# MingyuKim87/Safe_Denoiser

Hardware: AMD Instinct MI355X
Metric: images/sec (512x512, 50 steps, SD-v1.4 + repellency) (higher is better)
Workload: dtype bf16; 1 GPU; README-default end to end (safree = svf = lra = true, safree_neg_prompt_config.json:26-28): token ids -> CLIP -> SAFREE projection -> DDPM 50 steps x UNet on 3 guidance branches with per-prompt text switching + safe_denoiser.yaml repellency (kernel_fast, M=515, sigma 3.15, scale .33, margin 1.6, window 780<=t<=1000) -> VAE decode -> uint8 512x512 images; SD-v1.4 UNet / CLIP / VAE with random weigh; guidance_branches=3, text_encoder_precision=bf16x3, prompts_per_batch=64, latent_repeat=3, renoise_draws_rank0=3520, parallelism=prompt-shard x1

## Files before the change

include/sdn.h:

```cpp
#ifndef SDN_H_
#define SDN_H_

#include <stddef.h>
#include <stdint.h>

#ifdef __cplusplus
extern "C" {
#endif

#define SDN_OK            0
#define SDN_E_INVALID    -1
#define SDN_E_LAUNCH     -2
#define SDN_E_WORKSPACE  -3
#define SDN_E_ARCH       -4

int sdn_abi_version(void);
const char* sdn_device_arch_host(void);


#define SDN_REPEL_RBF     0
#define SDN_REPEL_SPARSE  1
#define SDN_QNORM_NONE    0
#define SDN_QNORM_CHANNEL 1
#define SDN_OUT_REPELLED  0
// ... 67 lines not shown
#define SDN_ACT_GEGLU_TANH 5
#define SDN_ACT_GELU      7
#define SDN_OUT_BF16      0
#define SDN_OUT_F32       1
#define SDN_OUT_F32_NCHW  2

typedef struct sdn_gemm_desc {
  int32_t M, N, K;
  int32_t a_mode;
  int32_t K1;
  int32_t Hs, Ws, Cin;
  int32_t Ho, Wo, stride;
  int32_t upsample;
  int32_t act;
  int32_t out_kind;
  int32_t rows_per_batch;
  int32_t ld_rowbias;
  int32_t ld_rowgate;
  int32_t residual_bcast;
  int32_t n_valid;
  int32_t ldc;
  int32_t asym_pad;
  int32_t split_k;
  int32_t res_pre;
  int32_t x3_out;
  int32_t f32_stream;
} sdn_gemm_desc;

int sdn_gemm_bf16(const sdn_gemm_desc* d_host, const void* a, const void* a2, const void* w,
                  const float* bias, const float* rowbias, const float* rowgate, const void* residual, void* out,
                  void* stream);
int sdn_gemm_f16(const sdn_gemm_desc* d_host, const void* a, const void* a2, const void* w,
                 const float* bias, const float* rowbias, const float* rowgate, const void* residual, void* out,
                 void* stream);

int sdn_groupnorm_bf16(const void* x, const void* x2, int32_t batch, int32_t hw, int32_t c1, int32_t c2,
                       int32_t groups, float eps, int32_t silu, const float* gamma, const float* beta,
                       void* out, float* stats_ws, void* stream);
int sdn_groupnorm_f16(const void* x, const void* x2, int32_t batch, int32_t hw, int32_t c1, int32_t c2,
                      int32_t groups, float eps, int32_t silu, const float* gamma, const float* beta,
                      void* out, float* stats_ws, void* stream);

int sdn_layernorm_bf16(const void* x, int64_t rows, int32_t c, float eps, const float* gamma,
                       const float* beta, void* out, void* stream);
int sdn_layernorm_f16(const void* x, int64_t rows, int32_t c, float eps, const float* gamma,
                      const float* beta, void* out, void* stream);

int sdn_attention_bf16(const void* q, const void* k, const void* v, void* out, int32_t batch, int32_t heads,
                       int32_t nq, int32_t nk, int32_t head_dim, int32_t ldq, int32_t ldk, int32_t ldv,
                       int32_t ldo, float scale, void* stream);
int sdn_attention_f16(const void* q, const void* k, const void* v, void* out, int32_t batch, int32_t heads,
                      int32_t nq, int32_t nk, int32_t head_dim, int32_t ldq, int32_t ldk, int32_t ldv,
                      int32_t ldo, float scale, void* stream);

typedef struct sdn_attn_segment2 {
  const void* q2; const void* k2; const void* v2; void* out2;
  int32_t n1, ldq2, ldk2, ldv2, ldo2;
} sdn_attn_segment2;
int sdn_joint_attention(int32_t dtype, const void* q, const void* k, const void* v, void* out,
                        const sdn_attn_segment2* seg2_host, int32_t batch, int32_t heads, int32_t n_total,
                        int32_t head_dim, int32_t ldq, int32_t ldk, int32_t ldv, int32_t ldo, float scale,
                        void* stream);

int sdn_layernorm_mod_bf16(const void* x, int64_t rows, int32_t c, float eps, const float* scale, const float* shift,
                           int32_t ld_mod, int32_t rows_per_batch, void* out, void* stream);
int sdn_layernorm_mod_f16(const void* x, int64_t rows, int32_t c, float eps, const float* scale, const float* shift,
                          int32_t ld_mod, int32_t rows_per_batch, void* out, void* stream);

int sdn_patchify_bf16(const float* latents, int32_t batch, int32_t c, int32_t h, int32_t w, int32_t p, void* out, void* stream);
int sdn_patchify_f16(const float* latents, int32_t batch, int32_t c, int32_t h, int32_t w, int32_t p, void* out, void* stream);
int sdn_unpatchify_f32(const float* tokens, int32_t batch, int32_t c, int32_t h, int32_t w, int32_t p, float* out, void* stream);

int sdn_conv_in_bf16(const float* latents_nchw, const void* w, const float* bias, int32_t batch, int32_t cin,
                     int32_t h, int32_t wd, int32_t cout, void* out_nhwc, void* stream);
int sdn_conv_in_f16(const float* latents_nchw, const void* w, const float* bias, int32_t batch, int32_t cin,
                    int32_t h, int32_t wd, int32_t cout, void* out_nhwc, void* stream);

int sdn_timestep_embed_bf16(float timestep, int32_t batch, int32_t dim, void* out, void* stream);
int sdn_timestep_embed_f16(float timestep, int32_t batch, int32_t dim, void* out, void* stream);

int sdn_gemm_f32(const sdn_gemm_desc* d_host, const void* a, const void* a2, const void* w,
                 const float* bias, const float* rowbias, const float* rowgate, const void* residual, void* out,
                 void* stream);
int sdn_groupnorm_f32(const void* x, const void* x2, int32_t batch, int32_t hw, int32_t c1, int32_t c2,
                      int32_t groups, float eps, int32_t silu, const float* gamma, const float* beta,
                      void* out, float* stats_ws, void* stream);
int sdn_layernorm_f32(const void* x, int64_t rows, int32_t c, float eps, const float* gamma,
                      const float* beta, void* out, void* stream);
int sdn_attention_f32(const void* q, const void* k, const void* v, void* out, int32_t batch, int32_t heads,
                      int32_t nq, int32_t nk, int32_t head_dim, int32_t ldq, int32_t ldk, int32_t ldv,
                      int32_t ldo, float scale, void* stream);
int sdn_conv_in_f32(const float* latents_nchw, const void* w, const float* bias, int32_t batch, int32_t cin,
                    int32_t h, int32_t wd, int32_t cout, void* out_nhwc, void* stream);
int sdn_timestep_embed_f32(float timestep, int32_t batch, int32_t dim, void* out, void* stream);

int sdn_gemm_x3(const sdn_gemm_desc* d_host, const void* a, const void* a2, const void* w,
                const float* bias, const float* rowbias, const float* rowgate, const void* residual, void* out,
                void* stream);
int sdn_attention_x3(const void* q, const void* k, const void* v, void* out, int32_t batch, int32_t heads,
                     int32_t nq, int32_t nk, int32_t head_dim, int32_t ldq, int32_t ldk, int32_t ldv,
                     int32_t ldo, float scale, void* stream);

int sdn_layernorm_mod_f32(const void* x, int64_t rows, int32_t c, float eps, const float* scale, const float* shift,
                          int32_t ld_mod, int32_t rows_per_batch, void* out, void* stream);
int sdn_patchify_f32(const float* latents, int32_t batch, int32_t c, int32_t h, int32_t w, int32_t p, void* out, void* stream);
int sdn_joint_attention_f32(int32_t mode, const void* q, const void* k, const void* v, void* out,
// ... 262 lines not shown
```

safe_denoiser_amd/_lib.py:

```python
from __future__ import annotations

import ctypes as C
import os

import torch

_HERE = os.path.dirname(os.path.abspath(__file__))
_LIB = None


class SdnUnavailable(RuntimeError):
    """libsdn.so is missing/unloadable, or there is no gfx950 device for a compute call."""


class SdnError(RuntimeError):
    """A libsdn entry point returned a negative status."""


_ERR = {-1: "SDN_E_INVALID (bad shape / null or misaligned pointer)", -2: "SDN_E_LAUNCH", -3: "SDN_E_WORKSPACE",
        -4: "SDN_E_ARCH"}


def lib_path() -> str:
    return os.environ.get("SDN_LIB", os.path.join(_HERE, "libsdn.so"))
# ... 148 lines not shown
    "sdn_vae_decode": (C.c_int, [_vp, _vp, _vp, _f32, _vp, _i32, _vp, _sz, _vp]),
    "sdn_vae_encoder_create": (C.c_int, [C.POINTER(VaeConfig), C.POINTER(_vp)]),
    "sdn_vae_encode": (C.c_int, [_vp, _vp, _vp, _vp, _i32, _vp, _sz, _vp]),
    "sdn_gaussian_sample": (C.c_int, [_vp, _vp, _i32, _i32, _i32, _f32, _vp, _vp]),
    "sdn_image_postprocess": (C.c_int, [_vp, _i32, _i32, _i32, _i32, _vp, _vp, _vp]),
    "sdn_latent_mix": (C.c_int, [_vp, _vp, _vp, _i32, _i32, _i32, _f32, _vp, _vp]),
    "sdn_softmax_rows": (C.c_int, [_i32, _vp, _i64, _i64, _i32, _f32, _vp, _i64, _vp]),
    "sdn_transpose16": (C.c_int, [_vp, _i32, _i32, _i64, _vp, _i64, _vp]),
    "sdn_clip_create": (C.c_int, [C.POINTER(ClipConfig), C.POINTER(_vp)]),
    "sdn_clip_forward": (C.c_int, [_vp, _vp, _vp, _vp, _vp, _i32, _vp, _sz, _vp]),
    "sdn_clip_embed": (C.c_int, [_i32, _vp, _vp, _vp, _i64, _i32, _i32, _i32, _vp, _vp]),
    "sdn_masked_attention": (C.c_int, [_i32, _vp, _vp, _vp, _vp, _vp, _i32, _i32, _i32, _i32, _i32, _i32, _i32, _i32, _i32,
                                       _f32, _vp]),
    "sdn_clip_proj_create": (C.c_int, [C.POINTER(ClipProjConfig), C.POINTER(_vp)]),
    "sdn_clip_proj_forward": (C.c_int, [_vp, _vp, _vp, _vp, _i64, _i64, _vp, _i64, _i32, _vp, _sz, _vp]),
    "sdn_clip_eos_rows": (C.c_int, [_i32, _vp, _vp, _vp, _vp, _i32, _i32, _i32, _i32, _i32, _f32, _vp, _vp, _vp]),
    "sdn_copy_rows_strided": (C.c_int, [_vp, _i32, _i32, _i32, _i32, _vp, _i64, _i64, _vp]),
    "sdn_clip_vision_create": (C.c_int, [C.POINTER(ClipVisionConfig), C.POINTER(_vp)]),
    "sdn_clip_vision_forward": (C.c_int, [_vp, _vp, _vp, _vp, _vp, _i32, _vp, _sz, _vp]),
    "sdn_clip_patch_rows": (C.c_int, [_i32, _vp, _i32, _i32, _i32, _i32, _vp, _vp]),
    "sdn_clip_vision_embed": (C.c_int, [_i32, _vp, _vp, _vp, _vp, _vp, _i32, _i32, _i32, _f32, _vp, _vp]),
    "sdn_clip_class_rows": (C.c_int, [_i32, _vp, _vp, _vp, _i32, _i32, _i32, _f32, _vp, _vp]),
    "sdn_image_resize_u8": (C.c_int, [_vp, _i32, _i32, _i32, _vp, _vp, _i32, _vp, _vp, _vp]),
    "sdn_clip_normalize_u8": (C.c_int, [_vp, _i32, _i32, _f32, _f32, _f32, _f32, _f32, _f32, _vp, _vp]),
    "sdn_image_resize_rect_u8": (C.c_int, [_vp, _i32, _i32, _i32, _i32, _i32, _vp, _vp, _i32, _vp, _vp, _i32, _vp, _vp, _vp, _f32, _f32,
                                           _f32, _f32, _f32, _f32, _vp]),
    "sdn_embed_row_scores": (C.c_int, [_vp, _i32, _i64, _vp, _i32, _i64, _i32, _i32, _i32, _i32, _f32, _f32, _vp, _vp]),
    "sdn_t5_create": (C.c_int, [C.POINTER(T5Config), C.POINTER(_vp)]),
    "sdn_t5_workspace_bytes": (_sz, [_vp, _i32, _i32]),
    "sdn_t5_flops": (C.c_double, [_vp, _i32, _i32, C.POINTER(C.c_double)]),
    "sdn_t5_forward": (C.c_int, [_vp, _vp, _vp, _vp, _i32, _vp, _i32, _vp, _sz, _vp]),
    "sdn_rmsnorm": (C.c_int, [_i32, _vp, _i32, _i64, _i32, _f32, _vp, _vp, _vp]),
    "sdn_embed_tokens": (C.c_int, [_i32, _vp, _vp, _i64, _i32, _i32, _vp, _vp]),
    "sdn_t5_bucket": (C.c_int, [_i32, _i32, _i32]),
    "sdn_t5_relative_bias": (C.c_int, [_i32, _vp, _i32, _i32, _i32, _i32, _vp, _vp]),
    "sdn_bias_attention": (C.c_int, [_i32, _vp, _vp, _vp, _vp, _vp, _vp, _i32, _i32, _i32, _i32, _i32, _i32, _i32, _i32, _f32,
                                     _vp]),
    "sdn_split3": (C.c_int, [_vp, _vp, _i64, _i32, _i32, _vp, _vp]),
    "sdn_expand3_weights": (C.c_int, [_vp, _i64, _i32, _i32, _vp, _vp]),
    "sdn_groupnorm_f32_triple": (C.c_int, [_vp, _vp, _i32, _i32, _i32, _i32, _i32, _f32, _i32, _vp, _vp, _vp, _vp, _vp]),
    "sdn_layernorm_f32_triple": (C.c_int, [_vp, _i64, _i32, _f32, _vp, _vp, _vp, _vp]),
    "sdn_attention_x3_triple": (C.c_int, [_vp, _vp, _vp, _vp, _i32, _i32, _i32, _i32, _i32, _i32, _i32, _i32, _i32, _f32, _vp]),
    "sdn_attention_x3_pairs": (C.c_int, [_vp, _vp, _vp, _i32, _i32, _vp, _i32, _i32, _i32, _i32, _i32, _i32, _i32, _i32, _i32, _f32, _i32, _vp]),
    "sdn_clip_embed_f32": (C.c_int, [_vp, _vp, _vp, _i64, _i32, _i32, _i32, _vp, _vp]),
    "sdn_masked_attention_f32": (C.c_int, [_vp, _vp, _vp, _vp, _vp, _i32, _i32, _i32, _i32, _i32, _i32, _i32, _i32, _i32, _f32, _vp]),
    "sdn_unet_prepare": (C.c_int, [_vp, _vp, _vp]),
    "sdn_unet_set_graph_mode": (None, [_vp, _i32]),
    "sdn_unet_set_text_version": (None, [_vp, C.c_uint64]),
    "sdn_unet_set_split_k": (None, [_vp, _i32]),
    "sdn_unet_set_conv_up4": (None, [_vp, _i32]),
    "sdn_conv_up4_weights": (C.c_int, [_i32, _vp, _i32, _i32, _vp, _vp]),
    "sdn_unet_profile_next": (None, [_vp]),
    "sdn_unet_profile_read": (C.c_int, [_vp, C.POINTER(ProfileRow), _i32]),
}


def lib():
    global _LIB
    if _LIB is None:
        path = lib_path()
        if not os.path.exists(path):
            raise SdnUnavailable(f"{path} not found: build it with `python -c 'import __graft_entry__ as g; g.build()'` "
                                 f"(or `make -C safe_denoiser_amd/csrc`).  There is no CPU fallback.")
        try:
            handle = C.CDLL(path)
        except OSError as e:
            raise SdnUnavailable(f"cannot load {path}: {e}") from e
        for name, (res, args) in SIGNATURES.items():
            fn = getattr(handle, name)
            fn.restype, fn.argtypes = res, args
        _LIB = handle
    return _LIB


def check(rc: int, what: str):
    if rc != 0:
        raise SdnError(f"{what} failed: {_ERR.get(rc, rc)}")


def require_gpu():
    if not torch.cuda.is_available():
        raise SdnUnavailable("no GPU visible: the safe-denoiser hot path only runs on an MI355X (gfx950); "
                             "there is no CPU fallback")


def dptr(t: torch.Tensor | None, dtype=None) -> int | None:
    if t is None:
        return None
    if not t.is_cuda:
        raise SdnUnavailable("tensor is not on the GPU: libsdn takes device pointers only (no CPU fallback)")
    if not t.is_contiguous():
        raise SdnError("tensor must be contiguous")
    if dtype is not None and t.dtype != dtype:
        raise SdnError(f"expected {dtype}, got {t.dtype}")
    return t.data_ptr()


def stream_ptr() -> int:
    return torch.cuda.current_stream().cuda_stream
```

safe_denoiser_amd/csrc/sdn_attn.hip:

```cpp
#include <stdlib.h>

#include <type_traits>

#include "sdn_common.h"
#include "sdn_ops.h"

namespace sdn_attn_detail {

typedef __attribute__((ext_vector_type(4))) short s16x4;
typedef __attribute__((ext_vector_type(16))) float f32x16;
typedef __attribute__((ext_vector_type(4))) unsigned int u32x4;

#if defined(__HIP_DEVICE_COMPILE__)
__device__ __forceinline__ __amdgpu_buffer_rsrc_t make_rsrc(const void* p, unsigned bytes) {
  return __builtin_amdgcn_make_buffer_rsrc(const_cast<void*>(p), 0, (int)bytes, 0x00020000);
}
typedef __attribute__((address_space(3))) void* lds_ptr_t;
#endif

#ifdef SDN_ATTN_STAMPS
#define SDN_ATS_DECL unsigned long long ats_prev = 0, ats_sum[7] = {0, 0, 0, 0, 0, 0, 0};
#define SDN_ATS_T0 unsigned long long ats_t0; asm volatile("s_memtime %0\n\ts_waitcnt lgkmcnt(0)" : "=s"(ats_t0)::"memory");
#define SDN_ATS_MARK(I)                                                                         \
  {                                                                                             \
// ... 802 lines not shown
          union { s16x4 hlf[2]; typename T::v8 full; } vfh, vfl;
          vfh.hlf[0] = __builtin_amdgcn_ds_read_tr16_b64_v4i16((__attribute__((address_space(3))) s16x4*)(pa));
          vfh.hlf[1] = __builtin_amdgcn_ds_read_tr16_b64_v4i16((__attribute__((address_space(3))) s16x4*)(pb));
          vfl.hlf[0] = __builtin_amdgcn_ds_read_tr16_b64_v4i16((__attribute__((address_space(3))) s16x4*)(la));
          vfl.hlf[1] = __builtin_amdgcn_ds_read_tr16_b64_v4i16((__attribute__((address_space(3))) s16x4*)(lb));
#pragma unroll
          for (int qs = 0; qs < QS; ++qs) o[qs][d] = T::mfma32(vfl.full, ph[qs], o[qs][d]);
#pragma unroll
          for (int qs = 0; qs < QS; ++qs) o[qs][d] = T::mfma32(vfh.full, pl[qs], o[qs][d]);
#pragma unroll
          for (int qs = 0; qs < QS; ++qs) o[qs][d] = T::mfma32(vfh.full, ph[qs], o[qs][d]);
        }
      }
    __builtin_amdgcn_s_setprio(0);
    asm volatile("s_waitcnt vmcnt(0)" ::: "memory");
    __syncthreads();
  }
#pragma unroll
  for (int qs = 0; qs < QS; ++qs) {
    float l_tot;
    if constexpr (ONES) {
      constexpr int row = HD % 32, ri = (row >> 3) * 4 + (row & 3);
      static_assert(((row >> 2) & 1) == 0, "ones row must live in lane half 0");
      l_tot = __shfl(o[qs][NDB - 1][ri], r, 64);
    } else {
      l_tot = l_run[qs] + __shfl_xor(l_run[qs], 32, 64);
    }
    const float inv = 1.f / l_tot;
    if (!qvalid[qs]) continue;
    const long qrow = (long)b * a.nq + q0 + 32 * qs + r;
#pragma unroll
    for (int d = 0; d < NDB; ++d)
#pragma unroll
      for (int tq = 0; tq < 4; ++tq) {
        const int dc = 32 * d + 8 * tq + 4 * h;
        if (dc < HD) {
          const float v0 = o[qs][d][4 * tq + 0] * inv, v1 = o[qs][d][4 * tq + 1] * inv, v2 = o[qs][d][4 * tq + 2] * inv, v3 = o[qs][d][4 * tq + 3] * inv;
          if (a.triple) {
            unsigned short* o3 = reinterpret_cast<unsigned short*>(a.out) + qrow * 3 * a.ldo + head * HD + dc;
            uint2 hi, lo;
            hi.x = T::pack2(v0, v1); hi.y = T::pack2(v2, v3);
            lo.x = T::pack2(v0 - T::to_f(hi.x & 0xffff), v1 - T::to_f(hi.x >> 16));
            lo.y = T::pack2(v2 - T::to_f(hi.y & 0xffff), v3 - T::to_f(hi.y >> 16));
            *reinterpret_cast<uint2*>(o3) = hi; *reinterpret_cast<uint2*>(o3 + a.ldo) = lo; *reinterpret_cast<uint2*>(o3 + 2 * a.ldo) = hi;
          } else {
            *reinterpret_cast<sdn_f32x4*>(reinterpret_cast<float*>(a.out) + qrow * a.ldo + head * HD + dc) = (sdn_f32x4){v0, v1, v2, v3};
          }
        }
      }
  }
#endif
}

static int g_attn_qs2 = 1;
static int g_attn_nomax = 1;

template <typename T, int HD>
int launch(const AttnArgs& a, int batch, int heads, hipStream_t st) {
  if (a.bias) {
    if constexpr (HD == 64) {
      if (a.q2 || a.causal) return SDN_E_INVALID;
      hipLaunchKernelGGL((k_attn<T, HD, false, true, true, 1, true>), dim3(a.nqb * a.npairs), dim3(THREADS), 0, st, a);
      return sdn_launch_status();
    } else {
      return SDN_E_INVALID;
    }
  }
  if (a.causal || a.kmask) {
    if constexpr (HD == 64) {
      if (a.q2) return SDN_E_INVALID;
      hipLaunchKernelGGL((k_attn<T, HD, false, true>), dim3(a.nqb * a.npairs), dim3(THREADS), 0, st, a);
      return sdn_launch_status();
    } else {
      return SDN_E_INVALID;
    }
  }
  if (a.q2) {
    if constexpr (HD == 64) {
      if (a.n1 % KV == 0 && a.ldk == a.ldk2 && a.ldv == a.ldv2) {
        hipLaunchKernelGGL((k_attn<T, HD, true, false, true>), dim3(a.nqb * a.npairs), dim3(THREADS), 0, st, a);
        return sdn_launch_status();
      }
    }
    hipLaunchKernelGGL((k_attn<T, HD, true>), dim3(a.nqb * a.npairs), dim3(THREADS), 0, st, a);
  } else {
    if constexpr (HD == 40) {
      if (a.nk > 2 * KV && a.nq >= 2 * QB && g_attn_qs2) {
        AttnArgs a2 = a;
        a2.nqb = (a.nq + 2 * QB - 1) / (2 * QB);
        hipLaunchKernelGGL((k_attn<T, HD, false, false, true, 2>), dim3(a2.nqb * a2.npairs), dim3(THREADS), 0, st, a2);
        return sdn_launch_status();
      }
    }
    hipLaunchKernelGGL((k_attn<T, HD, false>), dim3(a.nqb * a.npairs), dim3(THREADS), 0, st, a);
  }
  return sdn_launch_status();
}

static int g_attn_head_inner = 1;

template <typename T>
int run(const void* q, const void* k, const void* v, void* out, int32_t batch, int32_t heads, int32_t nq, int32_t nk,
        int32_t head_dim, int32_t ldq, int32_t ldk, int32_t ldv, int32_t ldo, float scale, void* stream,
        const sdn_attn_segment2* s2 = nullptr, int causal = 0, const int* kmask = nullptr, const float* bias = nullptr) {
  if (!q || !k || !v || !out || batch < 0 || heads <= 0 || nq <= 0 || nk <= 0) return SDN_E_INVALID;
  if ((ldq & 7) || (ldk & 7) || (ldv & 7) || (ldo & 3) || nk > 65535) return SDN_E_INVALID;
  if (ldq < heads * head_dim || ldk < heads * head_dim || ldv < heads * head_dim || ldo < heads * head_dim)
    return SDN_E_INVALID;
  auto al = [](const void* p, int n) { return (reinterpret_cast<uintptr_t>(p) & (n - 1)) == 0; };
  if (!al(q, 16) || !al(k, 16) || !al(v, 16) || !al(out, 8)) return SDN_E_INVALID;
  if (batch == 0) return SDN_OK;
  AttnArgs a{(const unsigned short*)q, (const unsigned short*)k, (const unsigned short*)v, (unsigned short*)out,
             nq, nk, ldq, ldk, ldv, ldo, scale * 1.4426950408889634f, heads, (nq + QB - 1) / QB, batch * heads,
             nullptr, nullptr, nullptr, nullptr, 0, 0, 0, 0, 0, 0, causal, kmask, g_attn_nomax, bias};
  if (!s2 && nk <= 2 * KV && (batch & 7) == 0 && g_attn_head_inner) a.head_inner = 1;
  if (causal && nq != nk) return SDN_E_INVALID;
  if (s2) {
    if (!s2->q2 || !s2->k2 || !s2->v2 || !s2->out2 || s2->n1 <= 0 || s2->n1 >= nq || nq != nk) return SDN_E_INVALID;
    if ((s2->ldq2 & 7) || (s2->ldk2 & 7) || (s2->ldv2 & 7) || (s2->ldo2 & 3)) return SDN_E_INVALID;
    if (!al(s2->q2, 16) || !al(s2->k2, 16) || !al(s2->v2, 16) || !al(s2->out2, 8)) return SDN_E_INVALID;
    a.q2 = (const unsigned short*)s2->q2; a.k2 = (const unsigned short*)s2->k2; a.v2 = (const unsigned short*)s2->v2;
    a.out2 = (unsigned short*)s2->out2; a.n1 = s2->n1;
    a.ldq2 = s2->ldq2; a.ldk2 = s2->ldk2; a.ldv2 = s2->ldv2; a.ldo2 = s2->ldo2;
  }
  hipStream_t st = (hipStream_t)stream;
  switch (head_dim) {
    case 40: return launch<T, 40>(a, batch, heads, st);
    case 64: return launch<T, 64>(a, batch, heads, st);
    case 80: return launch<T, 80>(a, batch, heads, st);
    case 160: return launch<T, 160>(a, batch, heads, st);
    default: return SDN_E_INVALID;
  }
}

}

#ifdef SDN_ATTN_STAMPS
extern "C" int sdn_debug_set_attn_stamps(void* p) {
  return (int)hipMemcpyToSymbol(HIP_SYMBOL(sdn_attn_detail::g_attn_stamps), &p, sizeof(p));
}
#endif
extern "C" void sdn_debug_set_attn_qs2(int on) { sdn_attn_detail::g_attn_qs2 = on; }
extern "C" void sdn_debug_set_attn_nomax(int on) { sdn_attn_detail::g_attn_nomax = on; }
extern "C" int sdn_attention_bf16(const void* q, const void* k, const void* v, void* out, int32_t batch,
                                  int32_t heads, int32_t nq, int32_t nk, int32_t head_dim, int32_t ldq,
                                  int32_t ldk, int32_t ldv, int32_t ldo, float scale, void* stream) {
  return sdn_attn_detail::run<SdnBF16>(q, k, v, out, batch, heads, nq, nk, head_dim, ldq, ldk, ldv, ldo, scale, stream);
}
extern "C" int sdn_attention_f16(const void* q, const void* k, const void* v, void* out, int32_t batch,
                                 int32_t heads, int32_t nq, int32_t nk, int32_t head_dim, int32_t ldq,
                                 int32_t ldk, int32_t ldv, int32_t ldo, float scale, void* stream) {
  return sdn_attn_detail::run<SdnF16>(q, k, v, out, batch, heads, nq, nk, head_dim, ldq, ldk, ldv, ldo, scale, stream);
}
extern "C" int sdn_joint_attention(int32_t dtype, const void* q, const void* k, const void* v, void* out,
                                   const sdn_attn_segment2* seg2, int32_t batch, int32_t heads, int32_t n_total,
                                   int32_t head_dim, int32_t ldq, int32_t ldk, int32_t ldv, int32_t ldo, float scale,
                                   void* stream) {
  if (!seg2) return SDN_E_INVALID;
  if (dtype == 1)
    return sdn_attn_detail::run<SdnF16>(q, k, v, out, batch, heads, n_total, n_total, head_dim, ldq, ldk, ldv, ldo, scale,
                                        stream, seg2);
  return sdn_attn_detail::run<SdnBF16>(q, k, v, out, batch, heads, n_total, n_total, head_dim, ldq, ldk, ldv, ldo, scale,
                                       stream, seg2);
}

extern "C" int sdn_masked_attention(int32_t dtype, const void* q, const void* k, const void* v, void* out,
                                    const int32_t* key_mask, int32_t causal, int32_t batch, int32_t heads, int32_t n,
                                    int32_t head_dim, int32_t ldq, int32_t ldk, int32_t ldv, int32_t ldo, float scale,
                                    void* stream) {
  if (!causal && !key_mask) return SDN_E_INVALID;
  if (dtype == 1)
    return sdn_attn_detail::run<SdnF16>(q, k, v, out, batch, heads, n, n, head_dim, ldq, ldk, ldv, ldo, scale, stream, nullptr,
                                        causal ? 1 : 0, key_mask);
  return sdn_attn_detail::run<SdnBF16>(q, k, v, out, batch, heads, n, n, head_dim, ldq, ldk, ldv, ldo, scale, stream, nullptr,
                                       causal ? 1 : 0, key_mask);
}

extern "C" int sdn_bias_attention(int32_t dtype, const void* q, const void* k, const void* v, void* out, const float* bias,
                                  const int32_t* key_mask, int32_t batch, int32_t heads, int32_t n, int32_t head_dim, int32_t ldq,
                                  int32_t ldk, int32_t ldv, int32_t ldo, float scale, void* stream) {
  if (!bias || (reinterpret_cast<uintptr_t>(bias) & 3) || n < 2 || n > 512 || head_dim != 64 || dtype < 0 || dtype > 1) return SDN_E_INVALID;
  if (dtype == 1)
    return sdn_attn_detail::run<SdnF16>(q, k, v, out, batch, heads, n, n, head_dim, ldq, ldk, ldv, ldo, scale, stream, nullptr, 0,
                                        key_mask, bias);
  return sdn_attn_detail::run<SdnBF16>(q, k, v, out, batch, heads, n, n, head_dim, ldq, ldk, ldv, ldo, scale, stream, nullptr, 0,
                                       key_mask, bias);
}

extern "C" void sdn_debug_set_attn_head_inner(int on) { sdn_attn_detail::g_attn_head_inner = on; }

extern "C" int sdn_attention_x3_pairs(const void* q, const void* k, const void* v, int32_t lo_offset_q, int32_t lo_offset_kv, void* out, int32_t batch,
                                      int32_t heads, int32_t nq, int32_t nk, int32_t head_dim, int32_t ldq, int32_t ldk, int32_t ldv,
                                      int32_t ldo, float scale, int32_t triple, void* stream) {
  using namespace sdn_attn_detail;
  if (!q || !k || !v || !out || batch < 0 || heads <= 0 || nq <= 0 || nk <= 0 || lo_offset_q <= 0 || lo_offset_kv <= 0) return SDN_E_INVALID;
  if ((ldq & 7) || (ldk & 7) || (ldv & 7) || (lo_offset_q & 7) || (lo_offset_kv & 7) || (ldo & 3) || nk > 65535) return SDN_E_INVALID;
  if (lo_offset_q < heads * head_dim || lo_offset_kv < heads * head_dim || ldq < lo_offset_q + heads * head_dim ||
      ldk < lo_offset_kv + heads * head_dim || ldv < lo_offset_kv + heads * head_dim || ldo < heads * head_dim)
    return SDN_E_INVALID;
  auto al = [](const void* p, int n) { return (reinterpret_cast<uintptr_t>(p) & (n - 1)) == 0; };
  if (!al(q, 16) || !al(k, 16) || !al(v, 16) || !al(out, 16)) return SDN_E_INVALID;
  if (head_dim != 40 && head_dim != 80 && head_dim != 160) return SDN_E_INVALID;
  if ((long)nk * ldk * 2 >= (1L << 31) || (long)nk * ldv * 2 >= (1L << 31)) return SDN_E_INVALID;
  if (batch == 0) return SDN_OK;
  static const int qs_env = getenv("SDN_X3P_QS") ? atoi(getenv("SDN_X3P_QS")) : 0;
  static const int nw_env = getenv("SDN_X3P_NW") ? atoi(getenv("SDN_X3P_NW")) : 0;
  int qs = (head_dim == 40 && nq >= 2 * QB) ? 2 : 1;
  int nw = (head_dim == 80 || head_dim == 160) && nq >= 2 * QB ? 8 : 4;
  if (head_dim == 40 && qs_env) qs = qs_env == 2 ? 2 : 1;
  if (nw_env) nw = nw_env == 8 ? 8 : 4;
  if (head_dim != 40) qs = 1;
  if (head_dim == 40 && qs == 2) nw = 4;
  const int qper = 32 * nw * qs;
  AttnPArgs a{(const unsigned short*)q, (const unsigned short*)k, (const unsigned short*)v, out, nq, nk, ldq, ldk, ldv, ldo, lo_offset_q, lo_offset_kv,
              scale * 1.4426950408889634f, heads, (nq + qper - 1) / qper, batch * heads, triple ? 1 : 0};
  const unsigned grid = (unsigned)(a.nqb * a.npairs);
  hipStream_t st = (hipStream_t)stream;
  if (head_dim == 40) {
    if (qs == 2) hipLaunchKernelGGL((k_attn_x3p<40, 2, 4, 64>), dim3(grid), dim3(256), 0, st, a);
    else if (nw == 8) hipLaunchKernelGGL((k_attn_x3p<40, 1, 8, 64>), dim3(grid), dim3(512), 0, st, a);
    else hipLaunchKernelGGL((k_attn_x3p<40, 1, 4, 64>), dim3(grid), dim3(256), 0, st, a);
  } else if (head_dim == 80) {
    if (nw == 8) hipLaunchKernelGGL((k_attn_x3p<80, 1, 8, 64>), dim3(grid), dim3(512), 0, st, a);
    else hipLaunchKernelGGL((k_attn_x3p<80, 1, 4, 64>), dim3(grid), dim3(256), 0, st, a);
  } else {
    if (nw == 8) hipLaunchKernelGGL((k_attn_x3p<160, 1, 8, 32>), dim3(grid), dim3(512), 0, st, a);
    else hipLaunchKernelGGL((k_attn_x3p<160, 1, 4, 32>), dim3(grid), dim3(256), 0, st, a);
  }
  return sdn_launch_status();
}
```

safe_denoiser_amd/csrc/sdn_ops.h:

```cpp
#pragma once
#include "../../include/sdn.h"

int sdn_gemm_pick_nrep(int n_padded, int act);
int sdn_gemm_pick_tile(int M, int N, int K, int act, int epilogue_reads = 0);

int sdn_temb_from_device(int dtype, const float* t_dev, int batch, int dim, void* out, void* stream);
int sdn_set_scalar(float* dst, float v, void* stream);

int sdn_gemm_pick_split(int M, int N, int K, int act, int out_kind);

int sdn_temb_f32(float timestep, const float* t_dev, int batch, int dim, void* out, void* stream);

int sdn_linear_pair_fold(int dtype, const void* wa, const void* wb, const float* ba, const float* bb, int C, int K, void* w_cat,
                         float* b_cat, void* stream);


int sdn_conv_slab_shape_ok(int M, int N, int Cin, int side, int stride, int upsample, int asym_pad, int out_kind, int n_valid);

int sdn_conv_up4_tile(int Hs, int Ws, int Cin, int N);

enum { SDN_NL_KERNEL, SDN_NL_DTYPE, SDN_NL_NQ, SDN_NL_R, SDN_NL_NCH, SDN_NL_CT, SDN_NL_NTILES, SDN_NL_ROWS_PER_TILE, SDN_NL_RPC,
       SDN_NL_NCHUNK, SDN_NL_STATS_SRC, SDN_NL_TRIPLE, SDN_NL_COUNT };
struct sdn_norm_launch { int kernel, dtype, nq, r, nch, ct, ntiles, rows_per_tile, rpc, nchunk, stats_src, triple; };
void record_norm_launch(const sdn_norm_launch& l);
```

safe_denoiser_amd/csrc/sdn_plan_core.hip:

```cpp
#include <math.h>

#include "sdn_plan.h"

namespace sdn_plan {

Ref Builder::param(const std::string& name, int kind, int rows, int cols, int rows_padded) {
  auto it = u->param_index.find(name);
  if (it != u->param_index.end()) return Ref{SP_W, u->params[it->second].offset};
  sdn_param_info pi;
  memset(&pi, 0, sizeof(pi));
  snprintf(pi.name, sizeof(pi.name), "%s", name.c_str());
  pi.kind = kind; pi.rows = rows; pi.cols = cols; pi.rows_padded = rows_padded > rows ? rows_padded : rows;
  const int64_t esz = (kind == SDN_P_VEC_F32 || kind == SDN_P_GEGLU_VEC) ? 4 : es;
  const int64_t bytes = (int64_t)pi.rows_padded * (cols > 0 ? cols : 1) * esz;
  pi.offset = u->weight_bytes;
  u->weight_bytes += (bytes + 255) & ~(int64_t)255;
  u->param_index[name] = (int)u->params.size();
  u->params.push_back(pi);
  return Ref{SP_W, pi.offset};
}
Ref Builder::stacked(const std::vector<std::string>& names, int rows_each, int cols) {
  Ref first;
  int64_t expect = -1;
  for (size_t i = 0; i < names.size(); ++i) {
// ... 179 lines not shown
    snprintf(o.label, sizeof(o.label), "k_gemm<%d>", sdn_gemm_pick_tile(o.gd.M, n_pad, o.gd.K, SDN_ACT_NONE));
  push_gemm(o);
}
void Builder::finish_up4() {
  for (const Up4& p : up4_pending) {
    const std::string name = "up4@" + std::to_string((long long)p.w9);
    const bool fresh = u->param_index.find(name) == u->param_index.end();
    Ref d = derived(name, (int64_t)16 * p.N * p.Cin * 2);
    if (fresh) { sdn_unet::FoldJob j{p.w9, -1, -1, -1, d.off, -1, -1, p.N, p.Cin}; j.kind = 3; u->fold_jobs.push_back(j); }
    if (p.op >= 0) plan->ops[(size_t)p.op].w = d;
  }
  up4_pending.clear();
}
void Builder::groupnorm(const Act& x, const Act* x2, float eps, int silu, Ref gamma, Ref beta, const Act& out) {
  Op o; o.kind = OP_GN; o.a = R(x); if (x2) o.a2 = R(*x2);
  o.batch = B; o.hw = x.hw; o.c1 = x.C; o.c2 = x2 ? x2->C : 0; o.groups = u->cfg.norm_groups; o.eps = eps;
  o.silu = silu; o.w = gamma; o.bias = beta; o.out = R(out); o.aux = gn_stats;
  if (x3t) { o.tri_out = 1; tri.insert(out.off); }
  if (x.st_off >= 0 && (!x2 || x2->st_off >= 0)) {
    o.cols1 = Ref{SP_WS, x.st_off};
    if (x2) o.cols2 = Ref{SP_WS, x2->st_off};
  }
  o.bytes = 2.0 * (o.cols1.space != SP_NONE ? 2.0 : 3.0) * (double)B * x.hw * (o.c1 + o.c2);
  snprintf(o.label, sizeof(o.label), o.cols1.space != SP_NONE ? "k_gn_apply" : "k_gn_stats+apply");
  plan->ops.push_back(o);
}
void Builder::layernorm(const Act& x, Ref gamma, Ref beta, const Act& out) {
  Op o; o.kind = OP_LN; o.a = R(x); o.rows = (int64_t)B * x.hw; o.c1 = x.C; o.eps = 1e-5f; o.w = gamma; o.bias = beta;
  o.out = R(out);
  if (x3t) { o.tri_out = 1; tri.insert(out.off); }
  o.bytes = 2.0 * 2.0 * (double)o.rows * x.C;
  snprintf(o.label, sizeof(o.label), "k_layernorm");
  plan->ops.push_back(o);
}
void Builder::repeat(const Act& in, const Act& out, int rep) {
  Op o; o.kind = OP_REPEAT; o.a = R(in); o.out = R(out); o.rows = in.content; o.c1 = rep;
  o.bytes = (double)in.content * (1 + rep);
  snprintf(o.label, sizeof(o.label), "k_repeat");
  plan->ops.push_back(o);
}
void Builder::attention(Ref q, Ref k, Ref v, Ref out, int nq, int nk, int C, int ldq, int ldk, int ldv, bool kv_pairs) {
  Op o; o.kind = OP_ATTN; o.a = q; o.k = k; o.v = v; o.out = out; o.batch = B; o.heads = u->cfg.n_heads;
  o.nq = nq; o.nk = nk; o.hd = C / u->cfg.n_heads; o.ldq = ldq; o.ldk = ldk; o.ldv = ldv; o.ldo = C;
  o.scale = 1.0f / sqrtf((float)o.hd);
  if (x3t && out.space == SP_WS) { o.tri_out = 1; tri.insert(out.off); }
  if (q.space == SP_WS && pairs.count(q.off)) {
    o.pair_in = kv_pairs ? 2 : 1; pairs.erase(q.off);
  } else if (kv_pairs) {
    plan_bad = true;
  }
  const double f = 4.0 * (double)B * o.heads * (double)nq * (double)nk * (double)o.hd;
  o.flops = f;
  o.bytes = 2.0 * (double)B * C * (2.0 * nq + 2.0 * nk);
  snprintf(o.label, sizeof(o.label), "k_attn<%d>", o.hd);
  plan->ops.push_back(o);
  plan->flops += f; plan->attn_flops += f;
}

Plan* get_plan(sdn_unet* u, int batch, int n) {
  if (u->kind == T5 && n == 0) n = 512;
  const int key = u->kind == T5 ? batch * 1024 + n : batch;
  auto it = u->plans.find(key);
  if (it != u->plans.end()) return &it->second;
  if (u->kind == T5 && u->plans.size() >= 64) {
    u->plans.clear();
    u->profiled_batch = 0;
  }
  Plan& p = u->plans[key];
  p.batch = batch;
  Builder b{u, &p};
  b.B = batch;
  b.seq = n;
  b.es = u->dtype() >= 2 ? 4 : 2;
  b.x3t = u->kind == UNET && u->dtype() == 3 && u->x3_expand;
  switch (u->kind) {
    case UNET: b.build(); break;
    case MMDIT: b.build_mmdit(); break;
    case VAE_DECODER: b.build_vae(); break;
    case VAE_ENCODER: b.build_vae_encoder(); break;
    case CLIP: case CLIP_PROJ: b.build_clip(); break;
    case T5: b.build_t5(); break;
    case CLIP_VISION: b.build_clip_vision(); break;
  }
  return &p;
}

}
```

Before: 8.405 images/sec.

## Add head-grouped cross-attention kernel for short text key sequences

Adds k_attn_text, a specialised attention kernel for short key lengths (nk <= 2*KV, e.g. the 77 CLIP text tokens). Each block handles a 160-wide slice holding several heads, stages Q for all of them in LDS once, and prefetches the next head's K/V while the current head is computed. It also writes output through LDS with coalesced 16-byte stores. The aim is to cut launch and per-head overhead and make Q/output traffic more efficient for cross-attention, at the cost of a large new kernel with its own numerical fallback (a rerun pass when the row sum is out of range).

```diff
diff --git a/include/sdn.h b/include/sdn.h
--- a/include/sdn.h
+++ b/include/sdn.h
@@ -143,6 +143,8 @@
 int sdn_attention_f16(const void* q, const void* k, const void* v, void* out, int32_t batch, int32_t heads,
                       int32_t nq, int32_t nk, int32_t head_dim, int32_t ldq, int32_t ldk, int32_t ldv,
                       int32_t ldo, float scale, void* stream);
+void sdn_debug_set_attn_text(int on);
+int64_t sdn_debug_attn_text_launches(void);
 
 typedef struct sdn_attn_segment2 {
   const void* q2; const void* k2; const void* v2; void* out2;
diff --git a/safe_denoiser_amd/_lib.py b/safe_denoiser_amd/_lib.py
--- a/safe_denoiser_amd/_lib.py
+++ b/safe_denoiser_amd/_lib.py
@@ -224,6 +224,8 @@
     "sdn_conv_up4_weights": (C.c_int, [_i32, _vp, _i32, _i32, _vp, _vp]),
     "sdn_unet_profile_next": (None, [_vp]),
     "sdn_unet_profile_read": (C.c_int, [_vp, C.POINTER(ProfileRow), _i32]),
+    "sdn_debug_set_attn_text": (None, [C.c_int]),
+    "sdn_debug_attn_text_launches": (_i64, []),
 }
 
 
diff --git a/safe_denoiser_amd/csrc/sdn_attn.hip b/safe_denoiser_amd/csrc/sdn_attn.hip
--- a/safe_denoiser_amd/csrc/sdn_attn.hip
+++ b/safe_denoiser_amd/csrc/sdn_attn.hip
@@ -878,6 +878,409 @@
 #endif
 }
 
+[[maybe_unused]] constexpr int TSEG = 160;
+[[maybe_unused]] constexpr int TQSTR = TSEG * 2 + 16;
+
+template <typename T, int HD>
+__global__ void __launch_bounds__(THREADS)
+k_attn_text(const AttnArgs a) {
+#if defined(__HIP_DEVICE_COMPILE__)
+  constexpr int HPW = TSEG / HD;
+  static_assert(HPW * HD == TSEG && HPW >= 1 && HPW <= 4, "head dims 40 / 80 / 160");
+  constexpr int KQ = (HD + 15) / 16;
+  constexpr int NDB = (HD + 31) / 32;
+  constexpr bool ONES = (HD % 32) != 0;
+  constexpr bool OFFSET_FREE = T::kDtype == 0;
+  constexpr bool CENTRED = T::kDtype == 1 && (KQ * 16 > HD);
+  constexpr bool CENTRED_SUB = T::kDtype == 1 && !CENTRED;
+  static_assert(!CENTRED || ((HD % 32) != 0 && HD - 16 * (KQ - 1) == 8), "centred form: row sums by the ones column, column HD = element 0 of the h = 1 lanes");
+  constexpr int CH = HD / 8;
+  constexpr int KCH = HD == 40 ? 5 : CH + 1;
+  constexpr int VCH = HD == 40 ? SDN_ATTN_VCH40 : (HD == 160 ? 20 : 12);
+  constexpr int KSTR = KCH * 16, VSTR = VCH * 16;
+  constexpr int STAGE = KV * KSTR + KV * VSTR;
+  constexpr int ZOFF = 2 * STAGE;
+  constexpr int QOFF = ZOFF + 64;
+  constexpr int CPR = TSEG / 8;
+  constexpr int NQL = 32 * CPR / 64;
+  __shared__ __attribute__((aligned(1024))) unsigned char smem[QOFF + QB * TQSTR];
+  constexpr bool kLateDma = HD == 40;
+#ifdef SDN_ATTN_NO_ASM_TR
+  constexpr bool kAsmTr = false;
+#else
+  constexpr bool kAsmTr = true;
+#endif
+  const int tid = threadIdx.x, lane = tid & 63;
+  const int wid = __builtin_amdgcn_readfirstlane(tid >> 6);
+  const int r = lane & 31, h = lane >> 5;
+  const int ngrp = a.heads / HPW;
+  int b, qblk, grp;
+  {
+    const int id = blockIdx.x, batch = a.npairs / a.heads;
+    if ((batch & 7) == 0) {
+      const int x = id & 7, j = id >> 3;
+      grp = j % ngrp;
+      const int rest = j / ngrp;
+      qblk = rest % a.nqb; b = (rest / a.nqb) * 8 + x;
+    } else {
+      grp = id % ngrp;
+      const int rest = id / ngrp;
+      qblk = rest % a.nqb; b = rest / a.nqb;
+    }
+  }
+  const int q0 = qblk * QB + wid * 32;
+  const int ntiles = (a.nk + KV - 1) / KV;
+
+  if (tid < 8) *reinterpret_cast<unsigned*>(smem + ZOFF + tid * 4) = tid == 0 ? (T::pack2(1.0f, 0.0f) & 0xffffu) : 0u;
+  else if (tid < 12) *reinterpret_cast<unsigned*>(smem + ZOFF + 32 + (tid - 8) * 4) = 0u;
+
+  constexpr int NPIECE = (KCH + VCH + 3) / 4;
+  unsigned dma_off[NPIECE];
+#pragma unroll
+  for (int i = 0; i < NPIECE; ++i) {
+    const int p = wid + 4 * i;
+    const bool isv = p >= KCH;
+    const int e = (isv ? p - KCH : p) * 64 + lane;
+    const int rowc = isv ? VCH : KCH;
+    const int row = e / rowc, ch = e - row * rowc;
+    dma_off[i] = ch < CH ? (unsigned)(((long)row * (isv ? a.ldv : a.ldk) + ch * 8) * 2) : 0x80000000u;
+  }
+  auto dma_issue = [&](int buf, int head, int t) {
+    const long k0 = (long)t * KV;
+    const unsigned short* kb_ = a.k + ((long)b * a.nk + k0) * a.ldk + head * HD;
+    const unsigned short* vb_ = a.v + ((long)b * a.nk + k0) * a.ldv + head * HD;
+    const long rk = ((a.nk - k0 - 1) * a.ldk + HD) * 2, rv = ((a.nk - k0 - 1) * a.ldv + HD) * 2;
+    const __amdgpu_buffer_rsrc_t rs_k = make_rsrc(kb_, (unsigned)(rk > 0 ? rk : 0));
+    const __amdgpu_buffer_rsrc_t rs_v = make_rsrc(vb_, (unsigned)(rv > 0 ? rv : 0));
+#pragma unroll
+    for (int i = 0; i < NPIECE; ++i) {
+      const int p = wid + 4 * i;
+      if (p < KCH)
+        __builtin_amdgcn_raw_ptr_buffer_load_lds(rs_k, (lds_ptr_t)(smem + buf * STAGE + p * 1024), 16, dma_off[i], 0, 0, 0);
+      else if (p < KCH + VCH)
+        __builtin_amdgcn_raw_ptr_buffer_load_lds(rs_v, (lds_ptr_t)(smem + buf * STAGE + KV * KSTR + (p - KCH) * 1024), 16,
+                                                 dma_off[i], 0, 0, 0);
+    }
+  };
+  dma_issue(0, grp * HPW, 0);
+
+  unsigned char* sQ = smem + QOFF + (wid * 32) * TQSTR;
+  {
+    u32x4 qv[NQL];
+#pragma unroll
+    for (int i = 0; i < NQL; ++i) {
+      const int e = lane + 64 * i, rr = e / CPR, ch = e - rr * CPR;
+      const int row = min(q0 + rr, a.nq - 1);
+      qv[i] = *reinterpret_cast<const u32x4*>(a.q + ((long)b * a.nq + row) * a.ldq + grp * TSEG + ch * 8);
+    }
+#pragma unroll
+    for (int i = 0; i < NQL; ++i) {
+      const int e = lane + 64 * i, rr = e / CPR, ch = e - rr * CPR;
+      u32x4 v = q0 + rr < a.nq ? qv[i] : (u32x4){0u, 0u, 0u, 0u};
+      v.x = T::pack2(T::to_f(v.x & 0xffff) * a.c, T::to_f(v.x >> 16) * a.c);
+      v.y = T::pack2(T::to_f(v.y & 0xffff) * a.c, T::to_f(v.y >> 16) * a.c);
+      v.z = T::pack2(T::to_f(v.z & 0xffff) * a.c, T::to_f(v.z >> 16) * a.c);
+      v.w = T::pack2(T::to_f(v.w & 0xffff) * a.c, T::to_f(v.w >> 16) * a.c);
+      *reinterpret_cast<u32x4*>(sQ + rr * TQSTR + ch * 16) = v;
+    }
+  }
+  const unsigned zpad = T::pack2(0.f * a.c, 0.f * a.c);
+  asm volatile("s_waitcnt vmcnt(0)" ::: "memory");
+  __syncthreads();
+
+  typename T::v8 qf[KQ];
+  f32x16 o[NDB];
+  float l_tot;
+  const int gi = lane & 15, gq = gi >> 2, gp = gi & 3, gcol = 16 * ((lane >> 4) & 1);
+
+  auto run_pass = [&](auto safe_c, int head, int buf0, int head_next) __attribute__((always_inline)) {
+    constexpr bool safe = decltype(safe_c)::value;
+    float m_run = OFFSET_FREE ? 0.f : -1e30f, l_run = 0.f, m_hi = -1e30f;
+#pragma unroll
+    for (int d = 0; d < NDB; ++d)
+#pragma unroll
+      for (int i = 0; i < 16; ++i) o[d][i] = 0.f;
+    if constexpr (CENTRED) {
+      u32x4 v = *reinterpret_cast<u32x4*>(&qf[KQ - 1]);
+      if (h == 1) v.x &= 0xffff0000u;
+      qf[KQ - 1] = *reinterpret_cast<typename T::v8*>(&v);
+    }
+    for (int t = 0; t < ntiles; ++t) {
+      const int buf = (buf0 + t) & 1;
+      const unsigned char* sK = smem + buf * STAGE;
+      const unsigned char* sV = sK + KV * KSTR;
+      const bool more = t + 1 < ntiles;
+      const bool pre = more || head_next >= 0;
+      const int nh = more ? head : head_next, nt = more ? t + 1 : 0;
+      if (!kLateDma && pre) dma_issue(buf ^ 1, nh, nt);
+      const int nkb = a.nk - t * KV > 32 ? 2 : 1;
+
+      f32x16 st[2];
+      __builtin_amdgcn_s_setprio(1);
+#pragma unroll
+      for (int kb = 0; kb < 2; ++kb) {
+        if (kb < nkb) {
+#pragma unroll
+          for (int i = 0; i < 16; ++i) st[kb][i] = 0.f;
+#pragma unroll
+          for (int s = 0; s < KQ; ++s) {
+            const unsigned char* kp = sK + (32 * kb + r) * KSTR + (16 * s + 8 * h) * 2;
+            if (16 * s + 16 > HD) { if (16 * s + 8 * h >= HD) kp = smem + ZOFF + (CENTRED ? 0 : 16); }
+            const typename T::v8 kf = *reinterpret_cast<const typename T::v8*>(kp);
+            st[kb] = T::mfma32(kf, qf[s], st[kb]);
+          }
+        }
+      }
+      __builtin_amdgcn_s_setprio(0);
+      if (kLateDma && pre) dma_issue(buf ^ 1, nh, nt);
+      if ((t + 1) * KV > a.nk) {
+        const int k0 = t * KV;
+#pragma unroll
+        for (int kb = 0; kb < 2; ++kb)
+          if (kb < nkb) {
+#pragma unroll
+            for (int i = 0; i < 16; ++i) {
+              const int key = k0 + 32 * kb + (i & 3) + 8 * (i >> 2) + 4 * h;
+              if (key >= a.nk) st[kb][i] = -1e30f;
+            }
+          }
+      }
+      [[maybe_unused]] float mx = 0.f;
+      bool need_mx = safe;
+      if constexpr ((CENTRED || CENTRED_SUB) && !safe) need_mx = t == 0;
+      if (need_mx) {
+        if (nkb == 2) {
+          mx = fmaxf(st[0][0], st[1][0]);
+#pragma unroll
+          for (int i = 1; i < 16; ++i) mx = fmaxf(fmaxf(mx, st[0][i]), st[1][i]);
+        } else {
+          mx = st[0][0];
+#pragma unroll
+          for (int i = 1; i < 16; ++i) mx = fmaxf(mx, st[0][i]);
+        }
+        const unsigned u = __float_as_uint(mx);
+        const auto sw = __builtin_amdgcn_permlane32_swap(u, u, false, false);
+        mx = fmaxf(__uint_as_float(sw[0]), __uint_as_float(sw[1]));
+      }
+      if constexpr (OFFSET_FREE) {
+        constexpr float kGuard = 64.f;
+        m_hi = fmaxf(m_hi, mx);
+        const float drift = m_hi - m_run;
+        if (safe && __builtin_amdgcn_ballot_w64(fabsf(drift) > kGuard) != 0) {
+          const float m_new = fabsf(drift) > kGuard ? m_hi : m_run;
+          const float alpha = __builtin_amdgcn_exp2f(fminf(m_run - m_new, 126.f));
+          if (!ONES) l_run *= alpha;
+#pragma unroll
+          for (int d = 0; d < NDB; ++d)
+#pragma unroll
+            for (int i = 0; i < 16; ++i) o[d][i] *= alpha;
+          m_run = m_new;
+        }
+        if (safe && __builtin_amdgcn_ballot_w64(m_run != 0.f) != 0) {
+#pragma unroll
+          for (int kb = 0; kb < 2; ++kb)
+            if (kb < nkb) {
+#pragma unroll
+              for (int i = 0; i < 16; ++i) st[kb][i] = __builtin_amdgcn_exp2f(st[kb][i] - m_run);
+            }
+        } else {
+#pragma unroll
+          for (int kb = 0; kb < 2; ++kb)
+            if (kb < nkb) {
+#pragma unroll
+              for (int i = 0; i < 16; ++i) st[kb][i] = __builtin_amdgcn_exp2f(st[kb][i]);
+            }
+        }
+      } else {
+        if constexpr (!safe) {
+          if (t == 0) {
+            const unsigned o16 = T::pack2(mx, 0.f) & 0xffffu;
+            const float off = T::to_f(o16);
+            m_run = off;
+            if constexpr (CENTRED) {
+#pragma unroll
+              for (int kb = 0; kb < 2; ++kb)
+                if (kb < nkb) {
+#pragma unroll
+                  for (int i = 0; i < 16; ++i) st[kb][i] -= off;
+                }
+              u32x4 v = *reinterpret_cast<u32x4*>(&qf[KQ - 1]);
+              if (h == 1) v.x = (v.x & 0xffff0000u) | (o16 ^ 0x8000u);
+              qf[KQ - 1] = *reinterpret_cast<typename T::v8*>(&v);
+            }
+          }
+          const float sub = CENTRED_SUB ? m_run : 0.f;
+#pragma unroll
+          for (int kb = 0; kb < 2; ++kb)
+            if (kb < nkb) {
+#pragma unroll
+              for (int i = 0; i < 16; ++i) st[kb][i] = __builtin_amdgcn_exp2f(CENTRED_SUB ? st[kb][i] - sub : st[kb][i]);
+            }
+        } else {
+          const float m_new = fmaxf(m_run, mx);
+          if (__builtin_amdgcn_ballot_w64(m_new != m_run) != 0) {
+            const float alpha = __builtin_amdgcn_exp2f(m_run - m_new);
+            if (!ONES) l_run *= alpha;
+#pragma unroll
+            for (int d = 0; d < NDB; ++d)
+#pragma unroll
+              for (int i = 0; i < 16; ++i) o[d][i] *= alpha;
+            m_run = m_new;
+          }
+#pragma unroll
+          for (int kb = 0; kb < 2; ++kb)
+            if (kb < nkb) {
+#pragma unroll
+              for (int i = 0; i < 16; ++i) st[kb][i] = __builtin_amdgcn_exp2f(st[kb][i] - m_new);
+            }
+        }
+      }
+      if (!ONES) {
+        float ps = 0.f;
+        if (nkb == 2) {
+#pragma unroll
+          for (int i = 0; i < 16; ++i) ps += st[0][i] + st[1][i];
+        } else {
+#pragma unroll
+          for (int i = 0; i < 16; ++i) ps += st[0][i];
+        }
+        l_run += ps;
+      }
+      __builtin_amdgcn_s_setprio(1);
+#pragma unroll
+      for (int kb = 0; kb < 2; ++kb) {
+        if (kb < nkb) {
+          auto v_ptr = [&](int j, int half) -> const unsigned char* {
+            const int s2 = j / NDB, d = j % NDB;
+            const int keyb = 32 * kb + 16 * s2 + 4 * h + gq;
+            const unsigned char* pa = sV + keyb * VSTR + (32 * d + gcol + 4 * gp) * 2;
+            const unsigned char* pb = pa + 8 * VSTR;
+            if (32 * d + 32 > HD) {
+              const int col = 32 * d + gcol + 4 * gp;
+              if (col >= HD) pa = pb = smem + ZOFF + (ONES && col == HD ? 0 : 8);
+            }
+            return half ? pb : pa;
+          };
+          auto p_frag = [&](int s2) {
+            u32x4 pw;
+            pw.x = T::pack2(st[kb][8 * s2 + 0], st[kb][8 * s2 + 1]);
+            pw.y = T::pack2(st[kb][8 * s2 + 2], st[kb][8 * s2 + 3]);
+            pw.z = T::pack2(st[kb][8 * s2 + 4], st[kb][8 * s2 + 5]);
+            pw.w = T::pack2(st[kb][8 * s2 + 6], st[kb][8 * s2 + 7]);
+            return *reinterpret_cast<typename T::v8*>(&pw);
+          };
+          if constexpr (kAsmTr) {
+            auto v_addr = [&](int j, int half) -> unsigned {
+              return (unsigned)(uintptr_t)(__attribute__((address_space(3))) const unsigned char*)v_ptr(j, half);
+            };
+            s16x4 va[2][2];
+            asm volatile("ds_read_b64_tr_b16 %0, %1" : "=v"(va[0][0]) : "v"(v_addr(0, 0)));
+            asm volatile("ds_read_b64_tr_b16 %0, %1" : "=v"(va[0][1]) : "v"(v_addr(0, 1)));
+#pragma unroll
+            for (int j = 0; j < 2 * NDB; ++j) {
+              if (j + 1 < 2 * NDB) {
+                asm volatile("ds_read_b64_tr_b16 %0, %1" : "=v"(va[(j + 1) & 1][0]) : "v"(v_addr(j + 1, 0)));
+                asm volatile("ds_read_b64_tr_b16 %0, %1" : "=v"(va[(j + 1) & 1][1]) : "v"(v_addr(j + 1, 1)));
+                asm volatile("s_waitcnt lgkmcnt(2)" : "+v"(va[j & 1][0]), "+v"(va[j & 1][1]));
+              } else {
+                asm volatile("s_waitcnt lgkmcnt(0)" : "+v"(va[j & 1][0]), "+v"(va[j & 1][1]));
+              }
+              union { s16x4 hlf[2]; typename T::v8 full; } vf;
+              vf.hlf[0] = va[j & 1][0]; vf.hlf[1] = va[j & 1][1];
+              o[j % NDB] = T::mfma32(vf.full, p_frag(j / NDB), o[j % NDB]);
+            }
+          } else {
+#pragma unroll
+            for (int j = 0; j < 2 * NDB; ++j) {
+              union { s16x4 hlf[2]; typename T::v8 full; } vf;
+              vf.hlf[0] = __builtin_amdgcn_ds_read_tr16_b64_v4i16((__attribute__((address_space(3))) s16x4*)(v_ptr(j, 0)));
+              vf.hlf[1] = __builtin_amdgcn_ds_read_tr16_b64_v4i16((__attribute__((address_space(3))) s16x4*)(v_ptr(j, 1)));
+              o[j % NDB] = T::mfma32(vf.full, p_frag(j / NDB), o[j % NDB]);
+            }
+          }
+        }
+      }
+      __builtin_amdgcn_s_setprio(0);
+      asm volatile("s_waitcnt vmcnt(0)" ::: "memory");
+      if (more) __syncthreads();
+    }
+    if (ONES) {
+      constexpr int row = HD % 32;
+      constexpr int ri = (row >> 3) * 4 + (row & 3);
+      static_assert(((row >> 2) & 1) == 0, "ones row must live in lane half 0");
+      l_tot = __shfl(o[NDB - 1][ri], r, 64);
+    } else {
+      l_tot = l_run + __shfl_xor(l_run, 32, 64);
+    }
+    if constexpr (CENTRED || CENTRED_SUB) return !(l_tot >= 0x1p-10f && l_tot <= 0x1p15f);
+    else return !(l_tot >= 0x1p-64f && l_tot <= 0x1p64f);
+  };
+
+  int cur = 0;
+#pragma unroll 1
+  for (int hl = 0; hl < HPW; ++hl) {
+    const int head = grp * HPW + hl;
+    const int head_next = hl + 1 < HPW ? head + 1 : -1;
+    unsigned char* sQh = sQ + r * TQSTR + hl * HD * 2;
+#pragma unroll
+    for (int s = 0; s < KQ; ++s) {
+      const int dc = 16 * s + 8 * h;
+      u32x4 v = (u32x4){zpad, zpad, zpad, zpad};
+      if (dc < HD) v = *reinterpret_cast<const u32x4*>(sQh + dc * 2);
+      qf[s] = *reinterpret_cast<typename T::v8*>(&v);
+    }
+    bool rerun = true;
+    if (a.nomax) {
+      const bool bad = run_pass(std::false_type{}, head, cur, head_next);
+      volatile unsigned* flag = reinterpret_cast<volatile unsigned*>(smem + ZOFF + 32 + hl * 4);
+      if (__builtin_amdgcn_ballot_w64(bad) != 0 && lane == 0) *flag = 1u;
+      __syncthreads();
+      rerun = *flag != 0u;
+      cur = (cur + ntiles) & 1;
+      if (rerun) {
+        cur ^= 1;
+        dma_issue(cur, head, 0);
+        asm volatile("s_waitcnt vmcnt(0)" ::: "memory");
+        __syncthreads();
+      }
+    }
+    if (rerun) {
+      run_pass(std::true_type{}, head, cur, head_next);
+      __syncthreads();
+      cur = (cur + ntiles) & 1;
+    }
+    const float inv = 1.f / l_tot;
+#pragma unroll
+    for (int d = 0; d < NDB; ++d)
+#pragma unroll
+      for (int tq = 0; tq < 4; ++tq) {
+        const int dc = 32 * d + 8 * tq + 4 * h;
+        if (dc < HD) {
+          uint2 pk;
+          pk.x = T::pack2(o[d][4 * tq + 0] * inv, o[d][4 * tq + 1] * inv);
+          pk.y = T::pack2(o[d][4 * tq + 2] * inv, o[d][4 * tq + 3] * inv);
+          *reinterpret_cast<uint2*>(sQh + dc * 2) = pk;
+        }
+      }
+    asm volatile("" ::: "memory");
+  }
+#pragma unroll
+  for (int i = 0; i < NQL; ++i) {
+    const int e = lane + 64 * i, rr = e / CPR, ch = e - rr * CPR;
+    const u32x4 v = *reinterpret_cast<const u32x4*>(sQ + rr * TQSTR + ch * 16);
+    if (q0 + rr < a.nq)
+      *reinterpret_cast<u32x4*>(a.out + ((long)b * a.nq + q0 + rr) * a.ldo + grp * TSEG + ch * 8) = v;
+  }
+#endif
+}
+
+static int g_attn_text = 1;
+static int64_t g_attn_text_launches = 0;
+static bool text_hd_on(int hd, int nq) {
+  if (g_attn_text == 2) return hd == 40 || hd == 80 || hd == 160;
+  return hd == 40 || (hd == 160 && nq >= QB);
+}
+
 static int g_attn_qs2 = 1;
 static int g_attn_nomax = 1;
 
@@ -924,6 +1327,11 @@
 }
 
 static int g_attn_head_inner = 1;
+
+static bool text_shape(int heads, int head_dim, int nq, int nk, int ldq, int ldo) {
+  if (!g_attn_text || !text_hd_on(head_dim, nq) || nk > 2 * KV) return false;
+  return ldq == heads * head_dim && ldo == ldq && heads % (TSEG / head_dim) == 0;
+}
 
 template <typename T>
 int run(const void* q, const void* k, const void* v, void* out, int32_t batch, int32_t heads, int32_t nq, int32_t nk,
@@ -950,6 +1358,14 @@
     a.ldq2 = s2->ldq2; a.ldk2 = s2->ldk2; a.ldv2 = s2->ldv2; a.ldo2 = s2->ldo2;
   }
   hipStream_t st = (hipStream_t)stream;
+  if (!s2 && !causal && !kmask && !bias && al(out, 16) && text_shape(heads, head_dim, nq, nk, ldq, ldo)) {
+    const unsigned grid = (unsigned)(batch * a.nqb * (heads / (TSEG / head_dim)));
+    if (head_dim == 40) hipLaunchKernelGGL((k_attn_text<T, 40>), dim3(grid), dim3(THREADS), 0, st, a);
+    else if (head_dim == 80) hipLaunchKernelGGL((k_attn_text<T, 80>), dim3(grid), dim3(THREADS), 0, st, a);
+    else hipLaunchKernelGGL((k_attn_text<T, 160>), dim3(grid), dim3(THREADS), 0, st, a);
+    ++g_attn_text_launches;
+    return sdn_launch_status();
+  }
   switch (head_dim) {
     case 40: return launch<T, 40>(a, batch, heads, st);
     case 64: return launch<T, 64>(a, batch, heads, st);
@@ -1014,6 +1430,11 @@
 }
 
 extern "C" void sdn_debug_set_attn_head_inner(int on) { sdn_attn_detail::g_attn_head_inner = on; }
+extern "C" void sdn_debug_set_attn_text(int on) { sdn_attn_detail::g_attn_text = on; }
+extern "C" int64_t sdn_debug_attn_text_launches(void) { return sdn_attn_detail::g_attn_text_launches; }
+int sdn_attn_text_shape(int heads, int head_dim, int nq, int nk, int ldq, int ldo) {
+  return sdn_attn_detail::text_shape(heads, head_dim, nq, nk, ldq, ldo) ? 1 : 0;
+}
 
 extern "C" int sdn_attention_x3_pairs(const void* q, const void* k, const void* v, int32_t lo_offset_q, int32_t lo_offset_kv, void* out, int32_t batch,
                                       int32_t heads, int32_t nq, int32_t nk, int32_t head_dim, int32_t ldq, int32_t ldk, int32_t ldv,
diff --git a/safe_denoiser_amd/csrc/sdn_ops.h b/safe_denoiser_amd/csrc/sdn_ops.h
--- a/safe_denoiser_amd/csrc/sdn_ops.h
+++ b/safe_denoiser_amd/csrc/sdn_ops.h
@@ -23,3 +23,5 @@
        SDN_NL_NCHUNK, SDN_NL_STATS_SRC, SDN_NL_TRIPLE, SDN_NL_COUNT };
 struct sdn_norm_launch { int kernel, dtype, nq, r, nch, ct, ntiles, rows_per_tile, rpc, nchunk, stats_src, triple; };
 void record_norm_launch(const sdn_norm_launch& l);
+
+int sdn_attn_text_shape(int heads, int head_dim, int nq, int nk, int ldq, int ldo);
diff --git a/safe_denoiser_amd/csrc/sdn_plan_core.hip b/safe_denoiser_amd/csrc/sdn_plan_core.hip
--- a/safe_denoiser_amd/csrc/sdn_plan_core.hip
+++ b/safe_denoiser_amd/csrc/sdn_plan_core.hip
@@ -255,7 +255,8 @@
   const double f = 4.0 * (double)B * o.heads * (double)nq * (double)nk * (double)o.hd;
   o.flops = f;
   o.bytes = 2.0 * (double)B * C * (2.0 * nq + 2.0 * nk);
-  snprintf(o.label, sizeof(o.label), "k_attn<%d>", o.hd);
+  const bool text = es == 2 && !o.pair_in && !o.tri_out && sdn_attn_text_shape(o.heads, o.hd, nq, nk, ldq, o.ldo);
+  snprintf(o.label, sizeof(o.label), text ? "k_attn_text<%d>" : "k_attn<%d>", o.hd);
   plan->ops.push_back(o);
   plan->flops += f; plan->attn_flops += f;
 }
```

New measurement: 8.415 images/sec (median of 6 runs). Within noise of the previous version (+0.1%).
